# faltiska/Matcha-TTS-24k

Measured on AMD Instinct MI355X. Metric: mel-frames/s (100-bin, 24 kHz) end-to-end synthesise(), n_timesteps=10, higher is better.
Workload: dtype f32 via 2-term f16 split (fp32 accumulate)

## Files before the change

include/mtts.h:

```cpp
#ifndef MTTS_H
#define MTTS_H

#include <stddef.h>
#include <stdint.h>

#ifdef __cplusplus
extern "C" {
#endif

#define MTTS_ABI_VERSION 2
#define MTTS_IMAGE_REVISION 5

typedef struct mtts_ctx mtts_ctx;

typedef struct mtts_config {
    int32_t n_feats;
    int32_t n_spks;
    int32_t spk_emb_dim;
    int32_t n_vocab;
    int32_t enc_channels;
    int32_t enc_filter;
    int32_t enc_heads;
    int32_t enc_layers;
    int32_t enc_kernel;
// ... 59 lines not shown
                   float out_scale, float out_shift, void* d_ws, int64_t ws_bytes, void* stream);

int mtts_fold_rows(mtts_ctx* ctx, int y_max, int align);
int mtts_cfm_solve_folded(mtts_ctx* ctx, const float* d_x0, const float* d_mu, const int64_t* d_y_lengths, int y_max, int add_mu,
                          const float* h_t_span, int n_steps, int solver, int B, int T, int T_fold, float* d_out, int T_out,
                          float out_scale, float out_shift, void* d_ws, int64_t ws_bytes, void* stream);


int64_t mtts_gemm_packed_bytes(int N, int C, int ntaps);
int mtts_gemm_f32(const float* d_a, int lda, int B, int T_in, int C, int ntaps, const int* h_tap_off, int in_stride,
                  int T_out, const float* d_a_mask, const float* d_a_mean, const float* d_a_rstd, const float* d_a_part,
                  int a_nparts, const float* d_w,
                  void* d_wpacked, const float* d_bias, int N, int act, const float* d_p0, const float* d_p1,
                  const float* d_res, int ldr, const float* d_out_mask, float out_scale, float* d_out, int ldc,
                  float* d_stats_out, int terms, void* stream);

int64_t mtts_gemm_p16_scratch_bytes(int B, int T_in, int C, int T_out, int N);
int mtts_gemm_p16(const float* d_a, int lda, int B, int T_in, int C, int ntaps, const int* h_tap_off, int in_stride, int T_out,
                  const float* d_a_mask, const float* d_a_mean, const float* d_a_rstd, const float* d_a_part, int a_nparts,
                  const float* d_w, void* d_wpacked, const float* d_bias, int N, int act, const float* d_p0, const float* d_p1,
                  const float* d_res, int ldr, const float* d_out_mask, float out_scale, float* d_out, int ldc,
                  float* d_out16_f32, float out_lscale, float* d_stats_out, int force_bm, void* d_scratch, void* stream);

int mtts_attention_f32(const float* d_qkv, const float* d_mask, int B, int T, int H, int D, float scale, int mask_mode,
                       float* d_out, void* stream);

int mtts_attention_p16(const float* d_qkv, const float* d_mask, int B, int T, int H, int D, float scale, int mask_mode,
                       float* d_out, void* d_scratch, void* stream);

int64_t mtts_chain_stream_frags(int C, int inner, int ch, int n_qkv);
int mtts_chain_plan(int M, int ch, int* qb, int* prefetch_wgs);
int mtts_chain_stream_pack(int C, int inner, int ch, int n_qkv, const float* h_w_out, const float* h_w1, const float* h_w2,
                           const float* h_w_qkv, uint16_t* h_dst);
int64_t mtts_chain_stream_frags_pair(int C, int inner, int ch, int n_qkv);
int mtts_chain_stream_pack_pair(int C, int inner, int ch, int n_qkv, const float* h_w_out, const float* h_w1, const float* h_w2,
                                const float* h_w_qkv, uint16_t* h_dst);
int64_t mtts_tblock_chain_scratch_bytes(int M, int C, int inner, int n_qkv, int ch);
int mtts_tblock_chain(const float* d_att, const float* d_x, int M, int C, int inner, const float* h_w_out, const float* h_b_out,
                      const float* h_w1, const float* h_b1, const float* h_p0, const float* h_p1, const float* h_w2,
                      const float* h_b2, const float* h_w_qkv, const float* h_b_qkv, int n_qkv, const float* d_out_mask, int qb,
                      int ch, float* d_x_out, float* d_qkv_out, void* d_scratch, void* stream);
int mtts_tblock_chain_timed(const float* d_att, const float* d_x, int M, int C, int inner, const float* h_w_out, const float* h_b_out,
                            const float* h_w1, const float* h_b1, const float* h_p0, const float* h_p1, const float* h_w2,
                            const float* h_b2, const float* h_w_qkv, const float* h_b_qkv, int n_qkv, const float* d_out_mask,
                            int qb, int ch, float* d_x_out, float* d_qkv_out, void* d_scratch, void* stream, int repeat, float* h_ms);
int mtts_tblock_chain_pair_timed(const float* d_att, const float* d_x, int M, int C, int inner, const float* h_w_out, const float* h_b_out,
// ... 42 lines not shown
```

matcha-tts-24k_amd/_hip.py:

```python
from __future__ import annotations

import ctypes as C
import os
import subprocess
from pathlib import Path
from typing import Dict, Optional

import numpy as np
import torch

from .hparams import PathHParams

HERE = Path(__file__).resolve().parent
CSRC = HERE / "csrc"
LIB = Path(os.environ["MTTS_HIP_LIB"]) if os.environ.get("MTTS_HIP_LIB") else HERE / "libmtts_hip.so"
SOURCES = ["gemm_f32.hip", "attention_f32.hip", "gemm_p16.hip", "tblock_chain.hip", "norm_glue.hip", "vocos.hip", "model.hip"]
HEADERS = [CSRC / "kernels.h", CSRC / "device_utils.h", CSRC / "model.h", HERE.parent / "include" / "mtts.h"]
SOLVERS = {"euler": 0, "midpoint": 1, "rk4": 2}


class MttsConfig(C.Structure):
    _fields_ = [(n, C.c_int32) for n in (
        "n_feats", "n_spks", "spk_emb_dim", "n_vocab", "enc_channels", "enc_filter", "enc_heads", "enc_layers",
        "enc_kernel", "prenet_layers", "prenet_kernel", "dp_filter", "dp_kernel", "dp_layers", "dec_levels")] + [
        ("dec_channels", C.c_int32 * 4)] + [(n, C.c_int32) for n in (
            "dec_head_dim", "dec_heads", "dec_n_blocks", "dec_mid_blocks")]


def _deps(src: Path, seen=None):
    import re
    seen = set() if seen is None else seen
    if src in seen or not src.exists():
        return seen
    seen.add(src)
    for inc in re.findall(r'^\s*#\s*include\s+"([^"]+)"', src.read_text(), flags=re.M):
        _deps((src.parent / inc).resolve(), seen)
    return seen


# ... 65 lines not shown
        "mtts_destroy": (None, [vp]),
        "mtts_set_tensor": (i32, [vp, C.c_char_p, vp, i64]),
        "mtts_weights_bytes": (i64, [vp]),
        "mtts_upload_weights": (i32, [vp, vp, i64]),
        "mtts_debug_hold": (i32, [vp, i32]),
        "mtts_weights_signature": (i32, [vp, C.c_char_p, i64]),
        "mtts_export_weights": (i32, [vp, vp, i64, C.POINTER(i32)]),
        "mtts_import_weights": (i32, [vp, vp, i64, i32]),
        "mtts_encoder_workspace_bytes": (i64, [vp, i32, i32]),
        "mtts_text_encoder_forward": (i32, [vp, vp, vp, vp, vp, i32, i32, vp, vp, vp, vp, i64, vp]),
        "mtts_speaker_embedding": (i32, [vp, i32, vp, i32, vp, vp]),
        "mtts_durations": (i32, [vp, vp, f32, f32, i32, i32, vp, vp, vp, vp]),
        "mtts_durations_per_utterance": (i32, [vp, vp, vp, vp, i32, i32, vp, vp, vp, vp]),
        "mtts_align_pool": (i32, [vp, vp, vp, i32, i32, i32, i32, vp, vp, vp, vp]),
        "mtts_set_frame_limits": (i32, [vp, vp]),
        "mtts_decoder_workspace_bytes": (i64, [vp, i32, i32]),
        "mtts_decoder_forward": (i32, [vp, vp, vp, vp, f32, i32, i32, vp, vp, i64, vp]),
        "mtts_cfm_solve": (i32, [vp, vp, vp, vp, i32, vp, i32, i32, i32, i32, vp, i32, f32, f32, vp, i64, vp]),
        "mtts_fold_rows": (i32, [vp, i32, i32]),
        "mtts_cfm_solve_folded": (i32, [vp, vp, vp, vp, i32, i32, vp, i32, i32, i32, i32, i32, vp, i32, f32, f32, vp, i64, vp]),
        "mtts_gemm_packed_bytes": (i64, [i32, i32, i32]),
        "mtts_attention_p16": (i32, [vp, vp, i32, i32, i32, i32, f32, i32, vp, vp, vp]),
        "mtts_gemm_p16_scratch_bytes": (i64, [i32, i32, i32, i32, i32]),
        "mtts_gemm_p16": (i32, [vp, i32, i32, i32, i32, i32, vp, i32, i32, vp, vp, vp, vp, i32, vp, vp, vp, i32, i32, vp, vp, vp,
                                i32, vp, f32, vp, i32, vp, f32, vp, i32, vp, vp]),
        "mtts_gemm_f32": (i32, [vp, i32, i32, i32, i32, i32, vp, i32, i32, vp, vp, vp, vp, i32, vp, vp, vp, i32, i32, vp, vp, vp,
                                i32, vp, f32, vp, i32, vp, i32, vp]),
        "mtts_attention_f32": (i32, [vp, vp, i32, i32, i32, i32, f32, i32, vp, vp]),
        "mtts_chain_stream_frags": (i64, [i32, i32, i32, i32]),
        "mtts_chain_plan": (i32, [i32, i32, C.POINTER(C.c_int), C.POINTER(C.c_int)]),
        "mtts_chain_stream_frags_pair": (i64, [i32, i32, i32, i32]),
        "mtts_chain_stream_pack_pair": (i32, [i32, i32, i32, i32, vp, vp, vp, vp, vp]),
        "mtts_chain_stream_pack": (i32, [i32, i32, i32, i32, vp, vp, vp, vp, vp]),
        "mtts_tblock_chain_scratch_bytes": (i64, [i32, i32, i32, i32, i32]),
        "mtts_tblock_chain": (i32, [vp, vp, i32, i32, i32, vp, vp, vp, vp, vp, vp, vp, vp, vp, vp, i32, vp, i32, i32, vp, vp, vp, vp]),
        "mtts_tblock_chain_timed": (i32, [vp, vp, i32, i32, i32, vp, vp, vp, vp, vp, vp, vp, vp, vp, vp, i32, vp, i32, i32, vp, vp, vp, vp,
                                          i32, C.POINTER(C.c_float)]),
        "mtts_tblock_chain_pair_timed": (i32, [vp, vp, i32, i32, i32, vp, vp, vp, vp, vp, vp, vp, vp, vp, vp, i32, vp, i32, i32, vp, vp, vp, vp,
                                          i32, C.POINTER(C.c_float)]),
        "mtts_row_stats": (i32, [vp, i32, i32, i32, f32, vp, vp, vp]),
        "mtts_channel_layernorm": (i32, [vp, i32, i32, i32, vp, vp, f32, i32, vp, vp, vp, vp]),
        "mtts_groupnorm_scratch_bytes": (i64, [i32, i32, i32]),
        "mtts_groupnorm_mish": (i32, [vp, vp, vp, vp, i32, i32, i32, i32, f32, vp, vp, vp]),
        "mtts_vocos_create": (vp, [i32, i32, i32, i32, i32, i32]),
        "mtts_vocos_destroy": (None, [vp]),
        "mtts_vocos_set_tensor": (i32, [vp, C.c_char_p, vp, i64]),
# ... 350 lines not shown


def gemm_p16(a, w, bias=None, *, B, T_in, T_out=None, tap_off=None, in_stride=1, a_mask=None, a_mean=None, a_rstd=None,
             a_part=None, act=0, p0=None, p1=None, res=None, out_mask=None, out_scale=1.0, stats_out=False, want_f32=True,
             want_p16=False, lscale=2048.0, force_bm=0):
    lib = load()
    N, Cc = w.shape[0], w.shape[1]
    ntaps = w.shape[2] if w.dim() == 3 else 1
    T_out = T_in if T_out is None else T_out
    taps = (C.c_int * ntaps)(*(tap_off if tap_off is not None else [j - ntaps // 2 for j in range(ntaps)]))
    packed = torch.empty(lib.mtts_gemm_packed_bytes(N, Cc, ntaps), dtype=torch.uint8, device=a.device)
    scratch = torch.empty(lib.mtts_gemm_p16_scratch_bytes(B, T_in, Cc, T_out, N), dtype=torch.uint8, device=a.device)
    out = torch.empty(B * T_out, N, dtype=torch.float32, device=a.device) if want_f32 else None
    out16 = torch.empty(B * T_out, N, dtype=torch.float32, device=a.device) if want_p16 else None
    stats = torch.empty(B * T_out, N // 64, 2, dtype=torch.float32, device=a.device) if stats_out else None
    check(lib.mtts_gemm_p16(ptr(a), a.shape[1], B, T_in, Cc, ntaps, taps, in_stride, T_out, ptr(a_mask), ptr(a_mean), ptr(a_rstd),
                            ptr(a_part), a_part.shape[1] if a_part is not None else 0,
                            ptr(w.contiguous()), packed.data_ptr(), ptr(bias), N, act, ptr(p0), ptr(p1), ptr(res),
                            res.shape[1] if res is not None else 0, ptr(out_mask), float(out_scale), ptr(out), N,
                            ptr(out16), float(lscale), ptr(stats), force_bm, scratch.data_ptr(), stream_ptr()))
    return {"out": out, "out16": out16, "stats": stats}


def _host(t):
    if t is None:
        return None, None
    a = np.ascontiguousarray(t.detach().to("cpu", torch.float32).numpy())
    return a, a.ctypes.data


def tblock_chain(att, x, w_out, b_out, w1, b1, p0, p1, w2, b2, w_qkv=None, b_qkv=None, out_mask=None, qb=64, ch=128, repeat=0, pair=False):
    lib = load()
    M, Cc = x.shape
    inner = att.shape[1] if att is not None else 0
    n_qkv = w_qkv.shape[0] if w_qkv is not None else 0
    n = lib.mtts_tblock_chain_scratch_bytes(M, Cc, inner, n_qkv, ch)
    if n < 0:
        raise RuntimeError("mtts_tblock_chain: unsupported shape")
    scratch = torch.empty(n, dtype=torch.uint8, device=x.device)
    x_out = torch.empty(M, Cc, dtype=torch.float32, device=x.device)
    qkv = torch.empty(M, n_qkv, dtype=torch.float32, device=x.device) if n_qkv else None
    keep = [_host(t) for t in (w_out, b_out, w1, b1, p0, p1, w2, b2, w_qkv, b_qkv)]
    hp = [k[1] for k in keep]
    ms = C.c_float(0.0)
    check((lib.mtts_tblock_chain_pair_timed if pair else lib.mtts_tblock_chain_timed)(ptr(att), ptr(x), M, Cc, inner, hp[0], hp[1], hp[2], hp[3], hp[4], hp[5], hp[6], hp[7], hp[8], hp[9],
                                      n_qkv, ptr(out_mask), qb, ch, ptr(x_out), ptr(qkv), scratch.data_ptr(), stream_ptr(), repeat,
# ... 48 lines not shown
```

matcha-tts-24k_amd/csrc/kernels.h:

```cpp
#pragma once
#include <hip/hip_runtime.h>
#include <stdint.h>
#include <stdlib.h>

namespace mtts {

constexpr int GEMM_BM = 128;
constexpr int GEMM_BN = 128;
constexpr int GEMM_BK = 32;
constexpr int MAX_TAPS = 7;

static inline int round_up(int x, int m) { return (x + m - 1) / m * m; }

extern thread_local const char* g_kernel_tag;
static inline const char* tf(bool b) { return b ? "true" : "false"; }

enum Act { ACT_NONE = 0, ACT_RELU = 1, ACT_SILU = 2, ACT_SNAKE = 3, ACT_GELU = 4 };

struct GemmArgs {
    const float* a0 = nullptr;
    const float* a1 = nullptr;
    int lda0 = 0, lda1 = 0;
    int c0 = 0, c1 = 0;
    int ktap = 0;
// ... 79 lines not shown
void panel_bf16_host(const float* panel, size_t n, uint16_t* plane);
hipError_t launch_split_panel_f16(const float* panel, size_t n, void* planes, hipStream_t s);

struct AttnArgs {
    const float* qkv = nullptr;
    const float* mask = nullptr;
    float* out = nullptr;
    int B = 0, T = 0, H = 0, D = 0;
    float scale = 1.0f;
    int mask_mode = 0;
    const _Float16* qkv16 = nullptr; int ld16 = 0;
    _Float16* out16 = nullptr; int ldo16 = 0;
    float out_lscale = 2048.0f;
    const int* klen = nullptr;
    bool fast16 = false;
    unsigned int* range_flag = nullptr;
    bool half16 = false;
    bool bf16 = false;
};
hipError_t launch_attention(const AttnArgs& a, hipStream_t s);
static inline double attn_flops(const AttnArgs& a) { return 4.0 * double(a.B) * a.H * double(a.T) * a.T * a.D; }
static inline double attn_bytes(const AttnArgs& a) { return 4.0 * double(a.B) * a.T * 4.0 * a.H * a.D; }

constexpr int CHAIN_WAVES = 8;
struct ChainArgs {
    int M = 0;
    int C = 0;
    int inner = 0;
    const _Float16* att16 = nullptr;
    int ld_att = 0;
    const _Float16* x16 = nullptr;
    int ld_x = 0;
    const _Float16* wstream = nullptr;
    long stream_frags = 0;
    const float* consts = nullptr;
    const float* b_qkv = nullptr;
    const float* wsum_qkv = nullptr;
    int n_qkv = 0;
    _Float16* x_out = nullptr;
    int ld_out = 0;
    const float* x_out_mask = nullptr;
    _Float16* qkv16 = nullptr;
    int ld_qkv = 0;
    float eps = 1e-5f;
    unsigned int* range_flag = nullptr;
    int qb = 0, ch = 0;
// ... 115 lines not shown
```

matcha-tts-24k_amd/csrc/model.h:

```cpp
#pragma once
#include <atomic>
#include <map>
#include <string>
#include <vector>

#include "../../include/mtts.h"
#include "kernels.h"

namespace mtts {

void set_error(const std::string& msg);
const char* get_error();

struct Panel {
    size_t w = 0, b = 0;
    size_t w16 = 0;
    bool has_bias = false;
    size_t wsum = 0;
    size_t wh16 = 0;
    int N = 0, C = 0, ntaps = 1, ktap = 0;
};
struct Vec { size_t off = 0; int n = 0; };

struct ResnetW {
// ... 50 lines not shown

struct ProfRec { hipEvent_t e0, e1; int klass; double flops, bytes; std::string tag; };

}

struct mtts_ctx {
    mtts_config cfg;
    std::map<std::string, std::vector<float>> raw;
    std::vector<float> image;
    float* d_image = nullptr;
    bool packed = false, uploaded = false;
    int gemm_terms = 6;
    unsigned int* cur_flag = nullptr;
    bool weights_saturate = false;
    const int* d_tlen = nullptr;
    bool half16 = false;
    bool bf16 = false;
    bool half_now = false;
    bool fast16 = false;
    bool p16_on = true;
    bool chain_on = true;
    int chain_ch = 256;
    int chain_qb = 0;
    bool pair_on = true;
    unsigned int pair_epoch = 0;
    int chain_min_rows = 5761;
    mtts::DecW dec;
    mtts::EncW enc;
    std::atomic<bool> in_use{false};
    bool prof_on = false;
    std::vector<mtts::ProfRec> prof;
    std::vector<hipEvent_t> ev_pool;
    size_t ev_used = 0;
};

struct mtts_vocos {
    mtts_ctx base;
    int n_mels = 100, dim = 512, inter = 1536, layers = 8, n_fft = 1024, hop = 256;
    int ld_spec = 0, im_off = 0;
    mtts::VocosW w;
};
```

matcha-tts-24k_amd/csrc/model.hip:

```cpp
#include "model.h"

#include <cmath>
#include <cstdlib>
#include <cstring>
#include <time.h>

namespace mtts {

static thread_local std::string g_err;
void set_error(const std::string& m) { g_err = m; }
const char* get_error() { return g_err.c_str(); }

#define HIP_OK(expr)                                                                        \
    do {                                                                                    \
        hipError_t _e = (expr);                                                             \
        if (_e != hipSuccess) {                                                             \
            set_error(std::string(#expr) + ": " + hipGetErrorString(_e));                   \
            return -1;                                                                      \
        }                                                                                   \
    } while (0)
#define RET_IF(expr)          \
    do {                      \
        int _r = (expr);      \
        if (_r) return _r;    \
// ... 229 lines not shown
#endif
    slot = g_verify + 8 * (size_t)g_verify_n++;
    hipLaunchKernelGGL(chain_verify_kernel, dim3((unsigned)((n + 255) / 256)), dim3(256), 0, s,
                       reinterpret_cast<const uint4*>(b.x_out), reinterpret_cast<const uint4*>(b3.x_out), a.M, cpr, slot);
    return 0;
}
extern "C" int mtts_debug_verify_read(int* out, int max_slots) {
    if (!g_verify) return 0;
    (void)hipDeviceSynchronize();
    const int n = g_verify_n < max_slots ? g_verify_n : max_slots;
    (void)hipMemcpy(out, g_verify, (size_t)n * 8 * sizeof(int), hipMemcpyDeviceToHost);
    verify_reset();
    return n;
}
#endif
static int run_gn_apply(mtts_ctx* c, const GnApplyArgs& a0, hipStream_t s) {
    GnApplyArgs a = a0;
    a.range_flag = c->cur_flag;
    a.half16 = c->half_now && a.out16 != nullptr;
    a.bf16 = a.half16 && c->bf16;
    LAUNCH(c, 2, 0, s, launch_gn_apply(a, s));
    return 0;
}
static int begin_call(mtts_ctx* c, void* d_ws, hipStream_t s) {
    c->cur_flag = static_cast<unsigned int*>(d_ws);
    HIP_OK(launch_fill_cols(static_cast<float*>(d_ws), 1, 64, 0, 64, 0.f, s));
    return 0;
}

struct WS {
    char* base;
    size_t off = 0, cap;
    bool overflow = false;
    WS(void* p, size_t c) : base(static_cast<char*>(p)), cap(c) {}
    void* bytes(size_t n) {
        off = (off + 255) & ~size_t(255);
        void* r = base ? base + off : nullptr;
        off += n;
        if (base && off > cap) overflow = true;
        return r;
    }
    float* f(size_t n) { return static_cast<float*>(bytes(n * sizeof(float))); }
};

struct Packer {
    mtts_ctx* c;
// ... 500 lines not shown
}

static int gn_fuse_rows(const GemmArgs& a, int C, int G, int T) {
    static const bool on = [] { const char* e = getenv("MTTS_GN_FUSE"); return !(e && e[0] == '0'); }();
    if (!on || !a.a16_0 || a.fast16 || (C % 64) || (C % G) || (C / G) < 32 || ((C / G) & 7)) return 0;
    const int rows = gemm_p16_wave_rows(a);
    return T >= rows ? rows : 0;
}

static int conv_gn_stats(mtts_ctx* c, DecBufs& d, GemmArgs& a, int lvl, const Vec& gamma, const Vec& beta, const Vec& bias_stats,
                         GnApplyArgs& g, hipStream_t s) {
    const int B = a.B, T = a.T_out, C = a.N;
    a.out = d.Y; a.ldc = C;
    const int fr = gn_fuse_rows(a, C, 8, T);
    if (fr) { a.gn_stats = d.gns; a.gn_groups = 8; a.gn_nrows = d.nr(lvl); g.tile_stats = d.gns; g.tile_rows = fr; }
    RET_IF(run_gemm(c, a, s));
    if (!fr) LAUNCH(c, 2, 0, s, launch_gn_partial(d.Y, B, T, C, 8, d.gnp, s, d.nr(lvl)));
    g.y = d.Y; g.partial = d.gnp; g.gamma = W(c, gamma.off); g.beta = W(c, beta.off); g.mask = d.mask[lvl]; g.nrows = d.nr(lvl);
    if (d.folded) { g.nextra = d.ne(lvl); g.bias_stats = W(c, bias_stats.off); }
    g.B = B; g.T = T; g.C = C;
    return 0;
}

static int resnet_block(mtts_ctx* c, DecBufs& d, const ResnetW& r, const Actv& in0, const Actv& in1, int lvl, const float* tbias,
                        float* dst, bool emit_stats, hipStream_t s) {
    const int B = d.B, T = d.Tl[lvl], C = r.cout;
    float* x = d.stream(dst);
    GemmArgs a;
    panel_args(c, r.conv1, a); rows_plain(a, B, T); taps_centered(a, 3);
    bind_in(d, a, 0, in0);
    if (in1.p) bind_in(d, a, 1, in1);
    GnApplyArgs g1;
    RET_IF(conv_gn_stats(c, d, a, lvl, r.gn1_g, r.gn1_b, r.gn1_bs, g1, s));
    g1.chbias = tbias;
    bind_out(d, g1, d.H, C);
    RET_IF(run_gn_apply(c, g1, s));
    GemmArgs b;
    panel_args(c, r.conv2, b); rows_plain(b, B, T); taps_centered(b, 3);
    bind_in(d, b, 0, actv(d, d.H, C));
    GnApplyArgs g2;
    RET_IF(conv_gn_stats(c, d, b, lvl, r.gn2_g, r.gn2_b, r.gn2_bs, g2, s));
    GemmArgs rc;
    panel_args(c, r.res, rc); rows_plain(rc, B, T);
    bind_in(d, rc, 0, in0);
    if (in1.p) bind_in(d, rc, 1, in1);
    static const bool tail_on = [] { const char* e = getenv("MTTS_GN_TAIL"); return !(e && e[0] == '0'); }();
    if (tail_on && g2.tile_rows && T >= 2 * gemm_p16_wave_rows(rc)) {
        rc.gnr_y = d.Y; rc.gnr_stats = d.gns; rc.gnr_tile_rows = g2.tile_rows; rc.gnr_groups = 8;
        rc.gnr_gamma = g2.gamma; rc.gnr_beta = g2.beta; rc.gnr_mask = g2.mask;
        rc.gnr_nextra = g2.nextra; rc.gnr_bias_stats = g2.bias_stats;
        bind_out(d, rc, x, C);
        rc.stats_out = d.lnp;
        RET_IF(run_gemm(c, rc, s));
        return 0;
    }
    rc.out = d.Rr; rc.ldc = C;
    RET_IF(run_gemm(c, rc, s));
    g2.res = d.Rr; g2.ldr = C;
    bind_out(d, g2, x, C);
    if (emit_stats && (C % 64) == 0) g2.stats_out = d.lnp;
    RET_IF(run_gn_apply(c, g2, s));
    return 0;
}

static int transformer_block(mtts_ctx* c, DecBufs& d, const TBlockW& t, int C, int lvl, bool emit_stats, float* dst, hipStream_t s) {
    const mtts_config& g = c->cfg;
    const int B = d.B, T = d.Tl[lvl], M = B * T, inner = g.dec_heads * g.dec_head_dim;
    const bool fuse = (C % 64) == 0;
// ... 133 lines not shown
                bind_in(d, a, 0, cur);
                a.B = B; a.T_in = d.Tl[l]; a.T_out = d.Tl[l]; a.in_stride = 1;
                a.tap_off[0] = ph == 0 ? 0 : 1;
                a.tap_off[1] = ph == 0 ? -1 : 0;
                bind_out(d, a, d.bufA[l - 1], r.cout, d.mask[l - 1]);
                a.out_T = d.Tl[l - 1]; a.out_stride = 2; a.out_off = ph;
                RET_IF(run_gemm(c, a, s));
            }
            cur = actv(d, d.bufA[l - 1], r.cout, d.mask[l - 1]);
        } else {
            GemmArgs a;
            panel_args(c, D.up_last, a); rows_plain(a, B, d.Tl[l]); taps_centered(a, 3);
            bind_in(d, a, 0, cur);
            float* o2 = other(cur, l);
            bind_out(d, a, o2, r.cout, d.mask[l]);
            RET_IF(run_gemm(c, a, s));
            cur = actv(d, o2, r.cout, d.mask[l]);
        }
    }
    const int C0 = g.dec_channels[0], T = d.T;
    GemmArgs a;
    panel_args(c, D.final_conv, a); rows_plain(a, B, T); taps_centered(a, 3);
    bind_in(d, a, 0, cur);
    GnApplyArgs ga;
    RET_IF(conv_gn_stats(c, d, a, 0, D.fgn_g, D.fgn_b, D.fgn_bs, ga, s));
    bind_out(d, ga, d.H, C0);
    RET_IF(run_gn_apply(c, ga, s));
    GemmArgs p;
    panel_args(c, D.final_proj, p); rows_plain(p, B, T);
    bind_in(d, p, 0, actv(d, d.H, C0));
    p.out_mask = d.mask[0];
    p.out = fo.out; p.ldc = fo.ldc; p.res = fo.res; p.ldr = fo.ldr; p.out_scale = fo.scale;
    RET_IF(run_gemm(c, p, s));
    return 0;
}
static int decoder_eval(mtts_ctx* c, DecBufs& d, const float* xin, int ev, const FinalOut& fo, hipStream_t s) {
    c->half_now = d.ew == 1;
    const int r = unet_eval(c, d, xin, ev, fo, s);
    c->half_now = false;
    return r;
}

static int build_frames(mtts_ctx* c, DecBufs& d, const float* mask, const int64_t* y_len, int T_true, hipStream_t s) {
    d.T_true = T_true;
    d.folded = y_len != nullptr;
    d.tables = d.folded || c->d_tlen != nullptr;
    if (!d.folded)
        for (int l = 0; l < d.nl; ++l)
            LAUNCH(c, 2, 0, s, launch_mask_down(mask, d.B, d.T, 1 << l, d.mask[l], d.Tl[l], s));
    if (d.tables) {
// ... 41 lines not shown
    if (!cfg) { set_error("null config"); return nullptr; }
    const mtts_config& g = *cfg;
    std::string why;
    if (g.dec_levels < 1 || g.dec_levels > 4) why = "dec_levels must be 1..4";
    else if (g.n_feats <= 0 || (2 * g.n_feats) % 4) why = "n_feats must be even";
    else if ((g.enc_channels + g.spk_emb_dim) % g.enc_heads) why = "encoder hidden size not divisible by heads";
    else if (((g.enc_channels + g.spk_emb_dim) / g.enc_heads) % 4 || (g.enc_channels + g.spk_emb_dim) / g.enc_heads > 64) why = "encoder head dim must be a multiple of 4, <= 64";
    else if (g.dec_head_dim % 4 || g.dec_head_dim > 64) why = "decoder head dim must be a multiple of 4, <= 64";
    else if (g.enc_channels % 4 || g.spk_emb_dim % 4 || g.enc_filter % 4 || g.dp_filter % 4) why = "channel counts must be multiples of 4";
    else if (g.enc_kernel > MAX_TAPS || g.prenet_kernel > MAX_TAPS || g.dp_kernel > MAX_TAPS) why = "kernel sizes above 5 unsupported";
    for (int i = 0; why.empty() && i < g.dec_levels; ++i)
        if (g.dec_channels[i] % 32) why = "decoder channels must be multiples of 32 (8 GroupNorm groups of 4k channels, K segments of 32)";
    if (!why.empty()) { set_error(why); return nullptr; }
    mtts_ctx* c = new mtts_ctx();
    c->cfg = g;
    c->gemm_terms = default_gemm_terms();
    { const char* e = getenv("MTTS_GEMM_TERMS"); c->fast16 = e && atoi(e) == 1; c->half16 = e && (atoi(e) == 16 || atoi(e) == 17); c->bf16 = e && atoi(e) == 17; }
    { const char* e = getenv("MTTS_P16"); c->p16_on = !(e && e[0] == '0'); }
    { const char* e = getenv("MTTS_CHAIN"); c->chain_on = !(e && e[0] == '0'); }
    { const char* e = getenv("MTTS_CHAIN_CH"); c->chain_ch = (e && atoi(e) == 128) ? 128 : 256; }
    { const char* e = getenv("MTTS_CHAIN_QB"); c->chain_qb = e ? atoi(e) : 0; }
    { const char* e = getenv("MTTS_CHAIN_MIN_ROWS"); if (e) c->chain_min_rows = atoi(e); }
    { const char* e = getenv("MTTS_CHAIN_PAIR"); c->pair_on = !(e && e[0] == '0'); }
    if (c->pair_on) {
        int dev = 0;
        hipDeviceProp_t prop;
        if (hipGetDevice(&dev) == hipSuccess && hipGetDeviceProperties(&prop, dev) == hipSuccess && prop.multiProcessorCount < 256) c->pair_on = false;
        (void)hipGetLastError();
    }
    return c;
}

int mtts_set_arithmetic(mtts_ctx* c, int terms) {
    if (!c) { set_error("null context"); return -1; }
    if (terms != 0 && terms != 1 && terms != 2 && terms != 3 && terms != 6 && terms != 16 && terms != 17) {
        set_error("mtts_set_arithmetic: terms must be 0, 1, 2, 3, 6, 16 or 17");
        return -1;
    }
    c->fast16 = terms == 1;
    c->half16 = terms == 16 || terms == 17;
    c->bf16 = terms == 17;
    c->gemm_terms = (terms == 1 || terms == 16 || terms == 17) ? 2 : terms;
    c->packed = false;
    c->uploaded = false;
    return 0;
}
// ... 437 lines not shown
    _Float16* a16 = reinterpret_cast<_Float16*>(sc);
    sc += (size_t)B * T_in * C * 4;
    _Float16* o16 = reinterpret_cast<_Float16*>(sc);
    sc += (size_t)B * T_out * round_up(N, 32) * 4;
    float* wsum = reinterpret_cast<float*>(sc);
    HIP_OK(launch_to_p16(d_a, lda, d_a_mask, B * T_in, C, C, a16, 2 * C, 2048.0f, s));
    hipLaunchKernelGGL(panel_rowsum_kernel, dim3((Np + 127) / 128), dim3(128), 0, s, static_cast<const float*>(d_wpacked), Np, Kp, wsum);
    HIP_OK(hipGetLastError());
    GemmArgs a;
    a.a16_0 = a16; a.lda16_0 = 2 * C; a.c0 = C; a.ktap = C; a.ntaps = ntaps;
    for (int j = 0; j < ntaps; ++j) a.tap_off[j] = h_tap_off ? h_tap_off[j] : 0;
    a.in_stride = in_stride; a.B = B; a.T_in = T_in; a.T_out = T_out;
    a.a_mean = d_a_mean; a.a_rstd = d_a_rstd; a.a_part = d_a_part; a.a_nparts = a_nparts; a.wsum = wsum;
    a.stats_out = d_stats_out;
    a.w16 = planes; a.terms = 2; a.bias = d_bias; a.N = N; a.act = act; a.p0 = d_p0; a.p1 = d_p1;
    a.res = d_res; a.ldr = ldr; a.out_mask = d_out_mask; a.out_scale = out_scale; a.out = d_out; a.ldc = ldc;
    if (d_out16_f32) { a.out16 = o16; a.ld16 = 2 * N; a.out_lscale = out_lscale; }
    a.out_T = T_out; a.out_stride = 1; a.out_off = 0; a.force_bm = force_bm;
    HIP_OK(launch_gemm(a, s));
    if (d_out16_f32) HIP_OK(launch_from_p16(o16, 2 * N, B * T_out, N, out_lscale, d_out16_f32, N, s));
    return 0;
}

int mtts_attention_f32(const float* d_qkv, const float* d_mask, int B, int T, int H, int D, float scale, int mask_mode, float* d_out,
                       void* stream) {
    AttnArgs a;
    a.qkv = d_qkv; a.mask = d_mask; a.out = d_out; a.B = B; a.T = T; a.H = H; a.D = D; a.scale = scale; a.mask_mode = mask_mode;
    HIP_OK(launch_attention(a, static_cast<hipStream_t>(stream)));
    return 0;
}

int mtts_attention_p16(const float* d_qkv, const float* d_mask, int B, int T, int H, int D, float scale, int mask_mode, float* d_out,
                       void* d_scratch, void* stream) {
    hipStream_t s = static_cast<hipStream_t>(stream);
    if (D != 64 || !d_scratch) { set_error("P16 attention needs D == 64 and a scratch buffer"); return -1; }
    const int M = B * T, C3 = 3 * H * D;
    _Float16* q16 = static_cast<_Float16*>(d_scratch);
    _Float16* o16 = q16 + (size_t)M * 2 * C3;
    HIP_OK(launch_to_p16(d_qkv, C3, nullptr, M, C3, C3, q16, 2 * C3, 1.0f, s));
    AttnArgs a;
    a.qkv16 = q16; a.ld16 = 2 * C3; a.out16 = o16; a.ldo16 = 2 * H * D; a.mask = d_mask;
    a.B = B; a.T = T; a.H = H; a.D = D; a.scale = scale; a.mask_mode = mask_mode;
    HIP_OK(launch_attention(a, s));
    HIP_OK(launch_from_p16(o16, 2 * H * D, M, H * D, a.out_lscale, d_out, H * D, s));
    return 0;
}
// ... 407 lines not shown
```

Measured before the change: 423,200.

## Fuse resnet conv1d with GroupNorm and Mish into one kernel

Adds a fused kernel that runs the 3-tap conv as an f16-split MFMA GEMM. One workgroup owns one batch row and one 48-channel group. It computes the GroupNorm statistics in LDS and applies the normalisation, Mish, mask and optional channel bias before writing split-f16 output. The decoder resnet blocks and the final block use it, when enabled by default, in place of the separate conv+stats GEMM and gn_apply kernels. This removes a launch and a round trip of the intermediate activation through global memory. In exchange it uses one workgroup per (batch, group), which can under-fill the GPU, and the gating heuristic tries to limit it to batch sizes that fill the chip.

After: 439,800, median of 6. +3.9%, better.

```diff
diff --git a/include/mtts.h b/include/mtts.h
--- a/include/mtts.h
+++ b/include/mtts.h
@@ -105,6 +105,11 @@
                   const float* d_res, int ldr, const float* d_out_mask, float out_scale, float* d_out, int ldc,
                   float* d_out16_f32, float out_lscale, float* d_stats_out, int force_bm, void* d_scratch, void* stream);
 
+int64_t mtts_conv_gn_scratch_bytes(int B, int T, int C, int N);
+int mtts_conv_gn(const float* d_x, int B, int T, int C, int c1, const float* d_w, void* d_wpacked, const float* d_bias, int N,
+                 const float* d_gamma, const float* d_beta, const float* d_mask, const float* d_chbias, const int* d_nrows,
+                 const int* d_nextra, const float* d_bias_stats, float eps, float* d_out, void* d_scratch, void* stream);
+
 int mtts_attention_f32(const float* d_qkv, const float* d_mask, int B, int T, int H, int D, float scale, int mask_mode,
                        float* d_out, void* stream);
 
diff --git a/matcha-tts-24k_amd/_hip.py b/matcha-tts-24k_amd/_hip.py
--- a/matcha-tts-24k_amd/_hip.py
+++ b/matcha-tts-24k_amd/_hip.py
@@ -14,7 +14,7 @@
 HERE = Path(__file__).resolve().parent
 CSRC = HERE / "csrc"
 LIB = Path(os.environ["MTTS_HIP_LIB"]) if os.environ.get("MTTS_HIP_LIB") else HERE / "libmtts_hip.so"
-SOURCES = ["gemm_f32.hip", "attention_f32.hip", "gemm_p16.hip", "tblock_chain.hip", "norm_glue.hip", "vocos.hip", "model.hip"]
+SOURCES = ["gemm_f32.hip", "attention_f32.hip", "gemm_p16.hip", "tblock_chain.hip", "resnet_conv.hip", "norm_glue.hip", "vocos.hip", "model.hip"]
 HEADERS = [CSRC / "kernels.h", CSRC / "device_utils.h", CSRC / "model.h", HERE.parent / "include" / "mtts.h"]
 SOLVERS = {"euler": 0, "midpoint": 1, "rk4": 2}
 
@@ -126,6 +126,8 @@
         "mtts_gemm_packed_bytes": (i64, [i32, i32, i32]),
         "mtts_attention_p16": (i32, [vp, vp, i32, i32, i32, i32, f32, i32, vp, vp, vp]),
         "mtts_gemm_p16_scratch_bytes": (i64, [i32, i32, i32, i32, i32]),
+        "mtts_conv_gn_scratch_bytes": (i64, [i32, i32, i32, i32]),
+        "mtts_conv_gn": (i32, [vp, i32, i32, i32, i32, vp, vp, vp, i32, vp, vp, vp, vp, vp, vp, vp, f32, vp, vp, vp]),
         "mtts_gemm_p16": (i32, [vp, i32, i32, i32, i32, i32, vp, i32, i32, vp, vp, vp, vp, i32, vp, vp, vp, i32, i32, vp, vp, vp,
                                 i32, vp, f32, vp, i32, vp, f32, vp, i32, vp, vp]),
         "mtts_gemm_f32": (i32, [vp, i32, i32, i32, i32, i32, vp, i32, i32, vp, vp, vp, vp, i32, vp, vp, vp, i32, i32, vp, vp, vp,
@@ -522,6 +524,17 @@
     return {"out": out, "out16": out16, "stats": stats}
 
 
+def conv_gn(x, w, bias, gamma, beta, mask, *, B, T, c1=0, chbias=None, nrows=None, nextra=None, bias_stats=None, eps=1e-5):
+    lib = load()
+    N, Cc = w.shape[0], w.shape[1]
+    packed = torch.empty(lib.mtts_gemm_packed_bytes(N, Cc, 3), dtype=torch.uint8, device=x.device)
+    scratch = torch.empty(lib.mtts_conv_gn_scratch_bytes(B, T, Cc, N), dtype=torch.uint8, device=x.device)
+    out = torch.empty(B * T, N, dtype=torch.float32, device=x.device)
+    check(lib.mtts_conv_gn(ptr(x), B, T, Cc, c1, ptr(w.contiguous()), packed.data_ptr(), ptr(bias), N, ptr(gamma), ptr(beta), ptr(mask),
+                           ptr(chbias), ptr(nrows), ptr(nextra), ptr(bias_stats), float(eps), ptr(out), scratch.data_ptr(), stream_ptr()))
+    return out
+
+
 def _host(t):
     if t is None:
         return None, None
diff --git a/matcha-tts-24k_amd/csrc/kernels.h b/matcha-tts-24k_amd/csrc/kernels.h
--- a/matcha-tts-24k_amd/csrc/kernels.h
+++ b/matcha-tts-24k_amd/csrc/kernels.h
@@ -125,6 +125,37 @@
 static inline double attn_flops(const AttnArgs& a) { return 4.0 * double(a.B) * a.H * double(a.T) * a.T * a.D; }
 static inline double attn_bytes(const AttnArgs& a) { return 4.0 * double(a.B) * a.T * 4.0 * a.H * a.D; }
 
+constexpr int CONV_GN_CPG = 48;
+constexpr int CONV_GN_MIN_ROWS = 65;
+constexpr int CONV_GN_SPLIT_ROWS = 192;
+constexpr int CONV_GN_MAX_ROWS = 384;
+struct ConvGnArgs {
+    const _Float16* a16_0 = nullptr;
+    const _Float16* a16_1 = nullptr;
+    int lda16_0 = 0, lda16_1 = 0;
+    int c0 = 0, c1 = 0;
+    const void* w16 = nullptr;
+    const float* bias = nullptr;
+    int B = 0, T = 0, N = 0;
+    const float* gamma = nullptr; const float* beta = nullptr;
+    const float* mask = nullptr;
+    const float* chbias = nullptr;
+    const int* nrows = nullptr;
+    const int* nextra = nullptr;
+    const float* bias_stats = nullptr;
+    float eps = 1e-5f;
+    _Float16* out16 = nullptr; int ld16 = 0;
+    const float* out16_mask = nullptr;
+    unsigned int* range_flag = nullptr;
+};
+bool conv_gn_supported(int T, int N);
+hipError_t launch_conv_gn(const ConvGnArgs& a, hipStream_t s);
+static inline double conv_gn_flops(const ConvGnArgs& a) { return 2.0 * double(a.B) * a.T * a.N * 3.0 * (a.c0 + a.c1); }
+static inline double conv_gn_bytes(const ConvGnArgs& a) {
+    const double M = double(a.B) * a.T, kin = a.c0 + a.c1;
+    return 4.0 * (M * kin + double(a.N) * 3.0 * kin + M * a.N);
+}
+
 constexpr int CHAIN_WAVES = 8;
 struct ChainArgs {
     int M = 0;
diff --git a/matcha-tts-24k_amd/csrc/model.h b/matcha-tts-24k_amd/csrc/model.h
--- a/matcha-tts-24k_amd/csrc/model.h
+++ b/matcha-tts-24k_amd/csrc/model.h
@@ -96,6 +96,8 @@
     bool chain_on = true;
     int chain_ch = 256;
     int chain_qb = 0;
+    int resnet_fuse = 3;
+    int resnet_fuse_rows = mtts::CONV_GN_MAX_ROWS;
     bool pair_on = true;
     unsigned int pair_epoch = 0;
     int chain_min_rows = 5761;
diff --git a/matcha-tts-24k_amd/csrc/model.hip b/matcha-tts-24k_amd/csrc/model.hip
--- a/matcha-tts-24k_amd/csrc/model.hip
+++ b/matcha-tts-24k_amd/csrc/model.hip
@@ -275,6 +275,13 @@
     LAUNCH(c, 2, 0, s, launch_gn_apply(a, s));
     return 0;
 }
+static int run_conv_gn(mtts_ctx* c, const ConvGnArgs& a0, hipStream_t s) {
+    ConvGnArgs a = a0;
+    a.range_flag = c->cur_flag;
+    LAUNCHB(c, 0, conv_gn_flops(a), conv_gn_bytes(a), s, launch_conv_gn(a, s));
+    return 0;
+}
+
 static int begin_call(mtts_ctx* c, void* d_ws, hipStream_t s) {
     c->cur_flag = static_cast<unsigned int*>(d_ws);
     HIP_OK(launch_fill_cols(static_cast<float*>(d_ws), 1, 64, 0, 64, 0.f, s));
@@ -821,6 +828,25 @@
     return 0;
 }
 
+static bool block1d_fusable(const mtts_ctx* c, const DecBufs& d, int T, int C) {
+    if (!d.p16 || c->half_now || c->fast16 || !conv_gn_supported(T, C) || T > c->resnet_fuse_rows) return false;
+    if (c->resnet_fuse & 4) return true;
+    const int wgs = 8 * d.B;
+    return wgs <= 256 && wgs >= (T <= CONV_GN_SPLIT_ROWS ? 128 : 192);
+}
+
+static int block1d_fused(mtts_ctx* c, DecBufs& d, const GemmArgs& a, int lvl, const Vec& gamma, const Vec& beta, const Vec& bias_stats,
+                         const float* chbias, float* dst, hipStream_t s) {
+    ConvGnArgs f;
+    f.a16_0 = a.a16_0; f.lda16_0 = a.lda16_0; f.c0 = a.c0;
+    f.a16_1 = a.a16_1; f.lda16_1 = a.lda16_1; f.c1 = a.c1;
+    f.w16 = a.w16; f.bias = a.bias; f.B = a.B; f.T = a.T_out; f.N = a.N;
+    f.gamma = W(c, gamma.off); f.beta = W(c, beta.off); f.mask = d.mask[lvl]; f.chbias = chbias; f.nrows = d.nr(lvl);
+    if (d.folded) { f.nextra = d.ne(lvl); f.bias_stats = W(c, bias_stats.off); }
+    f.out16 = image(dst); f.ld16 = d.ew * a.N;
+    return run_conv_gn(c, f, s);
+}
+
 static int resnet_block(mtts_ctx* c, DecBufs& d, const ResnetW& r, const Actv& in0, const Actv& in1, int lvl, const float* tbias,
                         float* dst, bool emit_stats, hipStream_t s) {
     const int B = d.B, T = d.Tl[lvl], C = r.cout;
@@ -829,20 +855,33 @@
     panel_args(c, r.conv1, a); rows_plain(a, B, T); taps_centered(a, 3);
     bind_in(d, a, 0, in0);
     if (in1.p) bind_in(d, a, 1, in1);
-    GnApplyArgs g1;
-    RET_IF(conv_gn_stats(c, d, a, lvl, r.gn1_g, r.gn1_b, r.gn1_bs, g1, s));
-    g1.chbias = tbias;
-    bind_out(d, g1, d.H, C);
-    RET_IF(run_gn_apply(c, g1, s));
+    const bool fusable = block1d_fusable(c, d, T, C);
+    if (fusable && (c->resnet_fuse & 1)) {
+        RET_IF(block1d_fused(c, d, a, lvl, r.gn1_g, r.gn1_b, r.gn1_bs, tbias, d.H, s));
+    } else {
+        GnApplyArgs g1;
+        RET_IF(conv_gn_stats(c, d, a, lvl, r.gn1_g, r.gn1_b, r.gn1_bs, g1, s));
+        g1.chbias = tbias;
+        bind_out(d, g1, d.H, C);
+        RET_IF(run_gn_apply(c, g1, s));
+    }
     GemmArgs b;
     panel_args(c, r.conv2, b); rows_plain(b, B, T); taps_centered(b, 3);
     bind_in(d, b, 0, actv(d, d.H, C));
-    GnApplyArgs g2;
-    RET_IF(conv_gn_stats(c, d, b, lvl, r.gn2_g, r.gn2_b, r.gn2_bs, g2, s));
     GemmArgs rc;
     panel_args(c, r.res, rc); rows_plain(rc, B, T);
     bind_in(d, rc, 0, in0);
     if (in1.p) bind_in(d, rc, 1, in1);
+    if (fusable && (c->resnet_fuse & 2)) {
+        RET_IF(block1d_fused(c, d, b, lvl, r.gn2_g, r.gn2_b, r.gn2_bs, nullptr, d.Y, s));
+        bind_res(d, rc, d.Y, C);
+        bind_out(d, rc, x, C);
+        if (emit_stats && (C % 64) == 0) rc.stats_out = d.lnp;
+        RET_IF(run_gemm(c, rc, s));
+        return 0;
+    }
+    GnApplyArgs g2;
+    RET_IF(conv_gn_stats(c, d, b, lvl, r.gn2_g, r.gn2_b, r.gn2_bs, g2, s));
     static const bool tail_on = [] { const char* e = getenv("MTTS_GN_TAIL"); return !(e && e[0] == '0'); }();
     if (tail_on && g2.tile_rows && T >= 2 * gemm_p16_wave_rows(rc)) {
         rc.gnr_y = d.Y; rc.gnr_stats = d.gns; rc.gnr_tile_rows = g2.tile_rows; rc.gnr_groups = 8;
@@ -1022,10 +1061,14 @@
     GemmArgs a;
     panel_args(c, D.final_conv, a); rows_plain(a, B, T); taps_centered(a, 3);
     bind_in(d, a, 0, cur);
-    GnApplyArgs ga;
-    RET_IF(conv_gn_stats(c, d, a, 0, D.fgn_g, D.fgn_b, D.fgn_bs, ga, s));
-    bind_out(d, ga, d.H, C0);
-    RET_IF(run_gn_apply(c, ga, s));
+    if ((c->resnet_fuse & 1) && block1d_fusable(c, d, T, C0)) {
+        RET_IF(block1d_fused(c, d, a, 0, D.fgn_g, D.fgn_b, D.fgn_bs, nullptr, d.H, s));
+    } else {
+        GnApplyArgs ga;
+        RET_IF(conv_gn_stats(c, d, a, 0, D.fgn_g, D.fgn_b, D.fgn_bs, ga, s));
+        bind_out(d, ga, d.H, C0);
+        RET_IF(run_gn_apply(c, ga, s));
+    }
     GemmArgs p;
     panel_args(c, D.final_proj, p); rows_plain(p, B, T);
     bind_in(d, p, 0, actv(d, d.H, C0));
@@ -1113,6 +1156,8 @@
     { const char* e = getenv("MTTS_CHAIN_QB"); c->chain_qb = e ? atoi(e) : 0; }
     { const char* e = getenv("MTTS_CHAIN_MIN_ROWS"); if (e) c->chain_min_rows = atoi(e); }
     { const char* e = getenv("MTTS_CHAIN_PAIR"); c->pair_on = !(e && e[0] == '0'); }
+    { const char* e = getenv("MTTS_RESNET_FUSE"); if (e) c->resnet_fuse = atoi(e) & 7; }
+    { const char* e = getenv("MTTS_RESNET_FUSE_ROWS"); if (e) c->resnet_fuse_rows = atoi(e); }
     if (c->pair_on) {
         int dev = 0;
         hipDeviceProp_t prop;
@@ -1596,6 +1641,33 @@
     return 0;
 }
 
+int64_t mtts_conv_gn_scratch_bytes(int B, int T, int C, int N) { return (int64_t)B * T * (C + N) * 4 + 1024; }
+int mtts_conv_gn(const float* d_x, int B, int T, int C, int c1, const float* d_w, void* d_wpacked, const float* d_bias, int N,
+                 const float* d_gamma, const float* d_beta, const float* d_mask, const float* d_chbias, const int* d_nrows,
+                 const int* d_nextra, const float* d_bias_stats, float eps, float* d_out, void* d_scratch, void* stream) {
+    hipStream_t s = static_cast<hipStream_t>(stream);
+    if (!d_x || !d_w || !d_wpacked || !d_scratch || !d_out) { set_error("null buffer"); return -1; }
+    if (C <= 0 || (C % 32) || c1 < 0 || (c1 % 32) || c1 >= C) { set_error("mtts_conv_gn: C and c1 must be multiples of 32, c1 < C"); return -1; }
+    if (!conv_gn_supported(T, N)) { set_error("mtts_conv_gn: unsupported shape (N = 384, 65 <= T <= 384)"); return -1; }
+    const int Np = round_up(N, GEMM_BN), Kp = 3 * C;
+    const size_t npanel = (size_t)Np * Kp;
+    float* planes = static_cast<float*>(d_wpacked) + ((npanel + 63) & ~size_t(63));
+    HIP_OK(launch_pack_weight(d_w, N, C, 3, static_cast<float*>(d_wpacked), s));
+    HIP_OK(launch_split_panel_f16(static_cast<const float*>(d_wpacked), npanel, planes, s));
+    _Float16* a16 = static_cast<_Float16*>(d_scratch);
+    _Float16* o16 = a16 + (size_t)B * T * C * 2;
+    HIP_OK(launch_to_p16(d_x, C, nullptr, B * T, C, C, a16, 2 * C, 2048.0f, s));
+    ConvGnArgs a;
+    a.a16_0 = a16; a.lda16_0 = 2 * C; a.c0 = C - c1;
+    if (c1) { a.a16_1 = a16 + 2 * (C - c1); a.lda16_1 = 2 * C; a.c1 = c1; }
+    a.w16 = planes; a.bias = d_bias; a.B = B; a.T = T; a.N = N;
+    a.gamma = d_gamma; a.beta = d_beta; a.mask = d_mask; a.chbias = d_chbias; a.nrows = d_nrows; a.nextra = d_nextra; a.bias_stats = d_bias_stats;
+    a.eps = eps; a.out16 = o16; a.ld16 = 2 * N;
+    HIP_OK(launch_conv_gn(a, s));
+    HIP_OK(launch_from_p16(o16, 2 * N, B * T, N, 2048.0f, d_out, N, s));
+    return 0;
+}
+
 int mtts_attention_f32(const float* d_qkv, const float* d_mask, int B, int T, int H, int D, float scale, int mask_mode, float* d_out,
                        void* stream) {
     AttnArgs a;
diff --git a/matcha-tts-24k_amd/csrc/resnet_conv.hip b/matcha-tts-24k_amd/csrc/resnet_conv.hip
--- /dev/null
+++ b/matcha-tts-24k_amd/csrc/resnet_conv.hip
@@ -0,0 +1,284 @@
+#include "kernels.h"
+#include "device_utils.h"
+#include <string>
+
+namespace mtts {
+
+using f32x4 = __attribute__((ext_vector_type(4))) float;
+using f16x8 = __attribute__((ext_vector_type(8))) _Float16;
+
+__device__ __attribute__((aligned(128))) _Float16 g_cg_zero_line[64];
+
+#define MTTS_CG_GLDS16(gp, lp) \
+    __builtin_amdgcn_global_load_lds((const __attribute__((address_space(1))) void*)(gp), (__attribute__((address_space(3))) void*)(lp), 16, 0, 0)
+
+constexpr int CG_NT = CONV_GN_CPG / 16;
+constexpr int CG_W_PIECES = CG_NT * 2;
+constexpr int CG_PS = CONV_GN_CPG + 4;
+static_assert(CG_NT == 3, "wave tiling below: 3 row tiles x 3 column tiles per wave");
+template <int KS>
+struct CgShape {
+    static constexpr int ROWS = KS == 2 ? CONV_GN_SPLIT_ROWS : CONV_GN_MAX_ROWS;
+    static constexpr int SLAB_PIECES = (ROWS + 2 + 7) / 8;
+    static constexpr int PIECES = SLAB_PIECES + 3 * CG_W_PIECES;
+    static constexpr int NJ = (PIECES + 7) / 8, NA = (SLAB_PIECES + 7) / 8;
+    static constexpr int STAGE = PIECES * 1024;
+    static constexpr int NST = KS == 2 ? 3 : 2;
+    static constexpr int RED = NST * STAGE;
+    static constexpr int LDS = RED + 256;
+    static constexpr int NPASS = ROWS / 64;
+    static_assert(ROWS == 48 * 8 / KS, "rows per wave");
+    static_assert(LDS <= 160 * 1024, "LDS per workgroup");
+    static_assert(ROWS * CG_PS * 4 <= RED, "the parked tile overlays the ring");
+};
+
+__device__ __forceinline__ void cg_wait_barrier(int n) {
+    switch (n) {
+        case 6: asm volatile("s_waitcnt vmcnt(6) lgkmcnt(0)\n\ts_barrier" ::: "memory"); break;
+        case 5: asm volatile("s_waitcnt vmcnt(5) lgkmcnt(0)\n\ts_barrier" ::: "memory"); break;
+        default: asm volatile("s_waitcnt vmcnt(0) lgkmcnt(0)\n\ts_barrier" ::: "memory"); break;
+    }
+}
+
+template <int SP, int NJ, int NA>
+__device__ __forceinline__ void cg_issue(char* st, int cc, int nc0, const _Float16* img0, const _Float16* img1, int ld0, int ld1,
+                                         const _Float16* wgrp, size_t wld, int tapk, int wv, int lane, int ch_a, int ch_w, const int (&ar)[NA]) {
+    const bool s1 = cc >= nc0;
+    const _Float16* img = (s1 ? img1 : img0) + (s1 ? cc - nc0 : cc) * 64;
+    const int ld = s1 ? ld1 : ld0;
+    const _Float16* wsrc = wgrp + cc * 64;
+#pragma unroll
+    for (int j = 0; j < NJ; ++j) {
+        const int q = wv + 8 * j;
+        if (q >= SP + 3 * CG_W_PIECES) continue;
+        const _Float16* src;
+        if (j < NA && q < SP) {
+            const int a = ar[j < NA ? j : 0];
+            src = a >= 0 ? img + (size_t)a * ld + ch_a : g_cg_zero_line + ch_a;
+        } else {
+            const int pw = q - SP, tap = pw / CG_W_PIECES, row = (pw - tap * CG_W_PIECES) * 8 + (lane >> 3);
+            src = wsrc + (size_t)row * wld + tap * tapk + ch_w;
+        }
+        MTTS_CG_GLDS16(src, st + q * 1024);
+    }
+}
+
+template <int KS>
+__global__ __launch_bounds__(512, 1) void conv_gn_kernel(const ConvGnArgs p) {
+    using S = CgShape<KS>;
+    extern __shared__ __attribute__((aligned(16))) char lds[];
+    const int tid = threadIdx.x, lane = tid & 63;
+    const int wv = __builtin_amdgcn_readfirstlane(tid >> 6);
+    const int ks = KS == 2 ? wv >> 2 : 0, wave = KS == 2 ? wv & 3 : wv;
+    int swz;
+    {
+        const int nwg = gridDim.x, id = blockIdx.x;
+        const int xcd = id & 7, q = nwg >> 3, r = nwg & 7;
+        swz = (xcd < r ? xcd * (q + 1) : r * (q + 1) + (xcd - r) * q) + (id >> 3);
+    }
+    const int b = swz >> 3, g = swz & 7;
+    const int T = p.T;
+    const int ktap = p.c0 + p.c1, Kp = 3 * ktap;
+    const int nstage = ktap >> 5;
+
+    const int ch_a = ((lane & 7) ^ (((wv & 1) * 4 + (lane >> 4)) & 7)) * 8;
+    const int ch_w = ((lane & 7) ^ ((((wv & 1) ^ (S::SLAB_PIECES & 1)) * 4 + (lane >> 4)) & 7)) * 8;
+    int arow[S::NA];
+#pragma unroll
+    for (int j = 0; j < S::NA; ++j) {
+        const int t = (wv + 8 * j) * 8 + (lane >> 3) - 1;
+        arow[j] = (unsigned)t < (unsigned)T ? b * T + t : -1;
+    }
+    const int my_pieces = (S::PIECES - wv + 7) >> 3;
+    auto issue = [&](int n, int slot) __attribute__((always_inline)) {
+        cg_issue<S::SLAB_PIECES, S::NJ, S::NA>(lds + slot * S::STAGE, n, p.c0 >> 5, p.a16_0, p.a16_1, p.lda16_0, p.lda16_1,
+                                               reinterpret_cast<const _Float16*>(p.w16) + (size_t)(g * CONV_GN_CPG) * Kp * 2, (size_t)Kp * 2, ktap * 2,
+                                               wv, lane, ch_a, ch_w, arow);
+    };
+
+    f32x4 acc[CG_NT][CG_NT], accx[CG_NT][CG_NT];
+#pragma unroll
+    for (int i = 0; i < 3; ++i)
+#pragma unroll
+        for (int j = 0; j < 3; ++j) { acc[i][j] = f32x4{0.f, 0.f, 0.f, 0.f}; accx[i][j] = acc[i][j]; }
+
+    const int fr = lane & 15, fq = lane >> 4;
+    const int f8w = (fr >> 1) & 7;
+    auto kstep = [&](const char* st, int u) __attribute__((always_inline)) {
+        const int R0 = wave * 48 + fr + u, f8a = (R0 >> 1) & 7;
+        const char* sa = st + R0 * 128;
+        const char* sw = st + S::SLAB_PIECES * 1024 + (u * CONV_GN_CPG + fr) * 128;
+        const int ah_o = (fq ^ f8a) * 16, al_o = ((4 + fq) ^ f8a) * 16, bh_o = (fq ^ f8w) * 16, bl_o = ((4 + fq) ^ f8w) * 16;
+        f16x8 ah[3], al[3];
+#pragma unroll
+        for (int i = 0; i < 3; ++i) {
+            ah[i] = *reinterpret_cast<const f16x8*>(sa + i * 16 * 128 + ah_o);
+            al[i] = *reinterpret_cast<const f16x8*>(sa + i * 16 * 128 + al_o);
+        }
+        f16x8 bh[3], bl[3];
+#pragma unroll
+        for (int j = 0; j < 3; ++j) {
+            bh[j] = *reinterpret_cast<const f16x8*>(sw + j * 16 * 128 + bh_o);
+            bl[j] = *reinterpret_cast<const f16x8*>(sw + j * 16 * 128 + bl_o);
+        }
+#pragma unroll
+        for (int i = 0; i < 3; ++i)
+#pragma unroll
+            for (int j = 0; j < 3; ++j) {
+                accx[i][j] = __builtin_amdgcn_mfma_f32_16x16x32_f16(ah[i], bl[j], accx[i][j], 0, 0, 0);
+                accx[i][j] = __builtin_amdgcn_mfma_f32_16x16x32_f16(al[i], bh[j], accx[i][j], 0, 0, 0);
+                acc[i][j] = __builtin_amdgcn_mfma_f32_16x16x32_f16(ah[i], bh[j], acc[i][j], 0, 0, 0);
+            }
+    };
+
+    constexpr int D = S::NST - 1;
+    issue(0, 0);
+    if (D > 1 && nstage > 1) issue(1, 1);
+    int slot = 0;
+    for (int n = 0; n < nstage; ++n) {
+        cg_wait_barrier(D > 1 && n + 1 < nstage ? my_pieces : 0);
+        if (n + D < nstage) issue(n + D, slot == 0 ? S::NST - 1 : slot - 1);
+        const char* st = lds + slot * S::STAGE;
+#pragma unroll
+        for (int u = 0; u < 3; ++u)
+            if (KS == 1 || ((n + u) & 1) == ks) kstep(st, u);
+        slot = slot == S::NST - 1 ? 0 : slot + 1;
+    }
+    __syncthreads();
+
+    float* P = reinterpret_cast<float*>(lds);
+    auto park = [&](bool add) __attribute__((always_inline)) {
+#pragma unroll
+        for (int i = 0; i < 3; ++i)
+#pragma unroll
+            for (int j = 0; j < 3; ++j)
+#pragma unroll
+                for (int r = 0; r < 4; ++r) {
+                    float* q = P + (wave * 48 + i * 16 + 4 * fq + r) * CG_PS + j * 16 + fr;
+                    float v = acc[i][j][r] + accx[i][j][r] * (1.0f / F16_RES_SCALE);
+                    if (add) v += q[0];
+                    q[0] = v;
+                }
+    };
+    if constexpr (KS == 2) {
+        if (ks == 1) park(false);
+        __syncthreads();
+        if (ks == 0) park(true);
+    } else park(false);
+
+    const int oct = tid & 7, c0g = g * CONV_GN_CPG + (oct < 6 ? oct : 0) * 8;
+    const bool live = oct < 6;
+    const f32x4 bi0 = *reinterpret_cast<const f32x4*>(p.bias + c0g), bi1 = *reinterpret_cast<const f32x4*>(p.bias + c0g + 4);
+    const f32x4 gm0 = *reinterpret_cast<const f32x4*>(p.gamma + c0g), gm1 = *reinterpret_cast<const f32x4*>(p.gamma + c0g + 4);
+    const f32x4 bt0 = *reinterpret_cast<const f32x4*>(p.beta + c0g), bt1 = *reinterpret_cast<const f32x4*>(p.beta + c0g + 4);
+    f32x4 cb0 = {0.f, 0.f, 0.f, 0.f}, cb1 = cb0;
+    if (p.chbias) { cb0 = *reinterpret_cast<const f32x4*>(p.chbias + c0g); cb1 = *reinterpret_cast<const f32x4*>(p.chbias + c0g + 4); }
+    const int nr = p.nrows ? max(0, min(T, p.nrows[b])) : T;
+    float x_ne = 0.f, x_bm = 0.f, x_bq = 0.f;
+    if (p.nextra) { x_ne = (float)p.nextra[b]; x_bm = p.bias_stats[2 * g]; x_bq = p.bias_stats[2 * g + 1]; }
+    float mk[S::NPASS], m16[S::NPASS];
+#pragma unroll
+    for (int it = 0; it < S::NPASS; ++it) {
+        const int row = it * 64 + (tid >> 3);
+        const bool in = row < T;
+        mk[it] = in ? p.mask[b * T + row] : 0.f;
+        m16[it] = in && p.out16_mask ? p.out16_mask[b * T + row] : 1.0f;
+    }
+    __syncthreads();
+
+    float v[S::NPASS][8];
+    float s = 0.f;
+#pragma unroll
+    for (int it = 0; it < S::NPASS; ++it) {
+        const int row = it * 64 + (tid >> 3);
+        const float* q = P + row * CG_PS + (live ? oct : 0) * 8;
+        const f32x4 a0 = *reinterpret_cast<const f32x4*>(q) + bi0, a1 = *reinterpret_cast<const f32x4*>(q + 4) + bi1;
+#pragma unroll
+        for (int e = 0; e < 4; ++e) { v[it][e] = a0[e]; v[it][4 + e] = a1[e]; }
+        if (live && row < nr) s += ((a0[0] + a0[1]) + (a0[2] + a0[3])) + ((a1[0] + a1[1]) + (a1[2] + a1[3]));
+    }
+    float* red = reinterpret_cast<float*>(lds + S::RED);
+    auto block_sum = [&](float x, float* slot8) __attribute__((always_inline)) {
+#pragma unroll
+        for (int off = 1; off < 64; off <<= 1) x += __shfl_xor(x, off);
+        if (lane == 0) slot8[wv] = x;
+        __syncthreads();
+        return ((slot8[0] + slot8[1]) + (slot8[2] + slot8[3])) + ((slot8[4] + slot8[5]) + (slot8[6] + slot8[7]));
+    };
+    float n = (float)(nr * CONV_GN_CPG);
+    const float total = block_sum(s, red);
+    float mean = n > 0.f ? total / n : 0.f;
+    float qd = 0.f;
+#pragma unroll
+    for (int it = 0; it < S::NPASS; ++it) {
+        const int row = it * 64 + (tid >> 3);
+        if (live && row < nr) {
+#pragma unroll
+            for (int e = 0; e < 8; ++e) { const float d = v[it][e] - mean; qd += d * d; }
+        }
+    }
+    float m2 = block_sum(qd, red + 8);
+    if (x_ne > 0.f) {
+        const float nb = x_ne * (float)CONV_GN_CPG, delta = x_bm - mean, nt = n + nb;
+        mean += delta * (nb / nt);
+        m2 += x_ne * x_bq + delta * delta * (n * nb / nt);
+        n = nt;
+    }
+    const float rs = n > 0.f ? 1.0f / sqrtf(m2 / n + p.eps) : 0.f;
+
+    bool range_bad = false;
+#pragma unroll
+    for (int it = 0; it < S::NPASS; ++it) {
+        const int row = it * 64 + (tid >> 3);
+        const bool in = row < T;
+        float o[8];
+#pragma unroll
+        for (int e = 0; e < 8; ++e) {
+            const float gme = e < 4 ? gm0[e & 3] : gm1[e & 3], bte = e < 4 ? bt0[e & 3] : bt1[e & 3];
+            o[e] = mish_f(((v[it][e] - mean) * rs) * gme + bte) * mk[it];
+            if (p.chbias) o[e] = (o[e] + (e < 4 ? cb0[e & 3] : cb1[e & 3])) * mk[it];
+        }
+        if (in && live) {
+            using f16x8s = __attribute__((ext_vector_type(8))) _Float16;
+            f16x8s hh, ll;
+            range_bad |= (out_of_f16_range(o[0], o[1], o[2], o[3]) || out_of_f16_range(o[4], o[5], o[6], o[7])) && m16[it] != 0.f;
+#pragma unroll
+            for (int e = 0; e < 8; ++e) {
+                _Float16 h, l;
+                split_f16(o[e] * m16[it], h, l);
+                hh[e] = h;
+                ll[e] = l;
+            }
+            _Float16* o16 = p.out16 + (size_t)(b * T + row) * p.ld16 + (c0g >> 5) * 64 + (c0g & 31);
+            *reinterpret_cast<f16x8s*>(o16) = hh;
+            *reinterpret_cast<f16x8s*>(o16 + 32) = ll;
+        }
+    }
+    raise_range_flag(p.range_flag, range_bad);
+}
+
+bool conv_gn_supported(int T, int N) { return N == 8 * CONV_GN_CPG && T >= CONV_GN_MIN_ROWS && T <= CONV_GN_MAX_ROWS; }
+
+hipError_t launch_conv_gn(const ConvGnArgs& a, hipStream_t s) {
+    if (a.B <= 0 || a.B > (1 << 20) || !conv_gn_supported(a.T, a.N)) return hipErrorInvalidValue;
+    if (!a.a16_0 || !a.w16 || !a.bias || !a.gamma || !a.beta || !a.mask || !a.out16) return hipErrorInvalidValue;
+    if (a.c0 <= 0 || (a.c0 & 31) || (a.c1 & 31) || a.c1 < 0 || (a.a16_1 == nullptr) != (a.c1 == 0)) return hipErrorInvalidValue;
+    if (a.lda16_0 < 2 * a.c0 || (a.lda16_0 & 7) || (a.a16_1 && (a.lda16_1 < 2 * a.c1 || (a.lda16_1 & 7)))) return hipErrorInvalidValue;
+    if (a.ld16 < 2 * a.N || (a.ld16 & 7)) return hipErrorInvalidValue;
+    if ((a.nextra != nullptr) != (a.bias_stats != nullptr)) return hipErrorInvalidValue;
+    const bool split = a.T <= CONV_GN_SPLIT_ROWS;
+    static bool configured[2] = {false, false};
+    const void* kern = split ? reinterpret_cast<const void*>(conv_gn_kernel<2>) : reinterpret_cast<const void*>(conv_gn_kernel<1>);
+    const int lds_bytes = split ? CgShape<2>::LDS : CgShape<1>::LDS;
+    if (!configured[split]) {
+        hipError_t e = hipFuncSetAttribute(kern, hipFuncAttributeMaxDynamicSharedMemorySize, lds_bytes);
+        if (e != hipSuccess) return e;
+        configured[split] = true;
+    }
+    g_kernel_tag = split ? "conv_gn_kernel<2>" : "conv_gn_kernel<1>";
+    if (split) hipLaunchKernelGGL(conv_gn_kernel<2>, dim3(8 * a.B), dim3(512), lds_bytes, s, a);
+    else hipLaunchKernelGGL(conv_gn_kernel<1>, dim3(8 * a.B), dim3(512), lds_bytes, s, a);
+    return hipGetLastError();
+}
+
+}
```
